# mourisl/centrifuger

Hardware: AMD Instinct MI355X
Metric: classified reads/sec (150 bp) (higher is better)
Workload: dtype u64; 1 GPU; 1.00 Gbp synthetic index (50x5x4 Mbp), 10000000 x 150 bp SE reads per step per GPU, -k 1, inputs resident in HBM; index_bp=1000000000, read_len=150, parallelism=reads sharded over 1 GPU(s), index replicated, no collective

## Files before the change

centrifuger_amd/csrc/cfr_device.hip:

```cpp
#include "cfr_device.hpp"

#include <hipcub/hipcub.hpp>
#include <chrono>

#include <algorithm>
#include <atomic>
#include <functional>
#include <cstdlib>
#include <cstring>
#include <thread>
#include <type_traits>

#include "cfr_hip_util.hpp"
#include "cfr_tail.hpp"
#include "cfr_kernels.hip.inc"

namespace cfr {

namespace {

inline const char *dbg_env(const char *name) {
  static const bool on = [] { const char *g = ::getenv("CFR_DEBUG_ENV"); return g && atoi(g) != 0; }();
  return on ? ::getenv(name) : nullptr;
}
// ... 551 lines not shown
      }
    } catch (const HipError &) {
      (void)hipGetLastError();
      (void)hipStreamSynchronize(stream_);
      for (void *q : tmp_here) temp_free(q);
      if (d_sa) (void)hipFree(d_sa);
      if (d_text_alloc) (void)hipFree(d_text_alloc);
      view_.sa32 = nullptr; view_.sa36 = nullptr; view_.text2 = nullptr; view_.text8 = nullptr; view_.text_min_l = 0;
      memset(&view_.steps, 0, sizeof(view_.steps));
    }
  }
  view_.loc_memo = nullptr;
  view_.memo_shift = 0;
  {
    const bool have_sa_now = have_sa();
    double budget_gb = opt.loc_memo_gb;
    if (budget_gb < 0) {
      budget_gb = fast_load ? 0.0 : 16.0;
      size_t free_b = 0, total_b = 0;
      if (!fast_load && hipMemGetInfo(&free_b, &total_b) == hipSuccess) budget_gb = std::max(have_sa_now ? 0.0 : budget_gb, ((double)free_b - 16e9) / 1e9);
      if (have_sa_now && (double)h.n * 4.0 > budget_gb * 1e9) budget_gb = 0;
    }
    if (const char *e = dbg_env("CFR_LOC_MEMO_GB")) budget_gb = atof(e);
    uint64_t max_val = h.adjusted_sa0;
    for (uint64_t x : h.selected_vals) max_val = std::max(max_val, x);
    if (protein && h.prot.end_marker_bits > 32) max_val = ~0ull;
    const bool fits32 = h.sampled_bits <= 32 && max_val <= 0xffffffffull;
    uint32_t shift = 0;
    while (shift < 8 && (double)((h.n >> shift) + 1) * 4.0 > budget_gb * 1e9) ++shift;
    if (budget_gb > 0 && fits32 && (1u << shift) < (uint32_t)h.sample_rate) try {
      const uint64_t entries = ((h.n - 1) >> shift) + 1;
      uint32_t *d_memo = dev_alloc<uint32_t>(entries);
      const unsigned gm = (unsigned)std::min<uint64_t>((entries + 255) / 256, 1u << 20);
      if (have_sa_now && view_.steps.pos && !(dbg_env("CFR_MEMO_WALK") && atoi(dbg_env("CFR_MEMO_WALK"))))
        k_memo_fill<<<gm, 256, 0, stream_>>>(view_, shift, entries, d_memo);
      else
        k_build_loc_memo<<<gm, 256, 0, stream_>>>(view_, shift, entries, d_memo);
      HIP_CHECK(hipGetLastError());
      HIP_CHECK(hipStreamSynchronize(stream_));
      view_.loc_memo = d_memo;
      view_.memo_shift = shift;
    } catch (const HipError &) { (void)hipGetLastError(); view_.loc_memo = nullptr; view_.memo_shift = 0; }
  }
  lap("locate memo");
  {
    size_t free_b = 0, total_b = 0;
    if (hipMemGetInfo(&free_b, &total_b) == hipSuccess) {
      const double budget = std::min(32e9, 0.4 * (double)free_b);
      piece_bases_max_ = (uint64_t)std::max(2.5e8, budget / 2.7);
    }
  }
  view_.max_entries = (uint64_t)(int64_t)(h.params.max_result * h.params.max_result_per_hit_factor);
  view_.locate_all = (h.params.max_result_per_hit_factor <= 0 || h.params.max_result <= 0) ? 1 : 0;
  d_view_ = dev_alloc<DevView>(1);
  HIP_CHECK(hipMemcpy(d_view_, &view_, sizeof(DevView), hipMemcpyHostToDevice));
}

DeviceIndex::~DeviceIndex() { release(); }

void DeviceIndex::release() {
  (void)hipSetDevice(device_);
  (void)hipDeviceSynchronize();
  for (void *p : owned_) (void)hipFree(p);
  owned_.clear();
  for (void *p : temps_) (void)hipFree(p);
  temps_.clear();
  for (auto &s : slots_) if (s.p) (void)hipFree(s.p);
  slots_.clear();
  if (pinned_) (void)hipHostFree(pinned_);
  pinned_ = nullptr; pinned_cap_ = 0;
  auto drop_event = [](hipEvent_t &e) { if (e) (void)hipEventDestroy(e); e = nullptr; };
  for (auto &set : evs_) for (auto &e : set) drop_event(e);
  for (auto &e : tail_done_) drop_event(e);
  for (auto &e : copy_done_) drop_event(e);
  for (auto &e : h2d_done_) drop_event(e);
  for (auto &e : copied_) drop_event(e);
  for (auto &e : search_done_) drop_event(e);
  for (auto &e : merge_ev_) drop_event(e);
  auto drop_stream = [](hipStream_t &s) { if (s) (void)hipStreamDestroy(s); s = nullptr; };
  drop_stream(tail_stream_);
  drop_stream(search2_stream_);
  if (prep_done_) { (void)hipEventDestroy(prep_done_); prep_done_ = nullptr; }
  drop_stream(h2d_stream_);
  drop_stream(dust_stream_);
  drop_stream(copy_stream_);
  drop_stream(stream_);
}

void *DeviceIndex::temp_alloc(size_t bytes) {
  void *p = nullptr;
  HIP_CHECK(hipMalloc(&p, std::max<size_t>(bytes, 16)));
  temps_.push_back(p);
  return p;
}
void DeviceIndex::temp_free(void *p) {
  if (!p) return;
  auto it = std::find(temps_.begin(), temps_.end(), p);
  if (it != temps_.end()) temps_.erase(it);
  (void)hipFree(p);
}

void DeviceIndex::rank_batch(const char *chars, const uint64_t *pos, const uint8_t *incl, size_t n, uint64_t *out_rank, char *out_access) {
  HIP_CHECK(hipSetDevice(device_));
  if (n == 0) return;
  char *d_c = (char *)scratch(S_P0, n);
  uint64_t *d_p = (uint64_t *)scratch(S_P1, n * 8);
// ... 763 lines not shown
    HIP_CHECK(hipStreamWaitEvent(copy_stream_, tail_done_[par], 0));
    static const bool no_copy = dbg_env("CFR_NO_COPY_OUT") && atoi(dbg_env("CFR_NO_COPY_OUT"));
    if (!no_copy) {
      HIP_CHECK(hipMemcpyAsync(reinterpret_cast<char *>(results) + lo * res_bytes, d_res, cnt * res_bytes, hipMemcpyDeviceToHost, copy_stream_));
      if (extent) HIP_CHECK(hipMemcpyAsync(reinterpret_cast<char *>(matches) + stride * lo * match_bytes, d_match, extent * match_bytes, hipMemcpyDeviceToHost, copy_stream_));
    }
    if (d_flag) HIP_CHECK(hipMemcpyAsync(h_flag, d_flag, kCtlWords * 8, hipMemcpyDeviceToHost, copy_stream_));
    HIP_CHECK(hipEventRecord(copy_done_[par], copy_stream_));
  };
  auto out_buffers = [&](size_t k, uint64_t extent, cfr_result *&d_res, cfr_match *&d_match, hipStream_t st) {
    const int par = (int)(k & 1);
    d_res = (cfr_result *)scratch(par ? S_RESULTS1 : S_RESULTS, std::max(pieces[k].second, sb) * sizeof(cfr_result));
    d_match = (cfr_match *)scratch(par ? S_MATCHES1 : S_MATCHES, (std::max<uint64_t>(extent, stride * sb) + 1) * sizeof(cfr_match));
    if (k >= 2) HIP_CHECK(hipStreamWaitEvent(st, copy_done_[par], 0));
  };

  std::vector<size_t> todo;
  for (size_t k = 0; k < nsub; ++k) todo.push_back(k);
  if (one_launch) {
    unsigned long long *pin = (unsigned long long *)pinned((2 + kCtlWords * kMaxSub + 3 * (kMaxSub + 1)) * 8);
    unsigned long long *pctl = pin + 2;
    for (size_t k = 0; k < kCtlWords * kMaxSub; ++k) pctl[k] = 0;
    if (!pool_cap_) pool_cap_ = std::max<uint64_t>(8ull * sb, 1ull << 20);
    const uint64_t pool_limit = std::max<uint64_t>(256ull * sb, 1ull << 26);
    for (int attempt = 0; attempt < 4 && !todo.empty(); ++attempt) {
      TailEntry *pool_e = (TailEntry *)scratch(S_POOL_E, pool_cap_ * sizeof(TailEntry));
      uint64_t *pool_v = (uint64_t *)scratch(S_POOL_V, pool_cap_ * 8);
      for (size_t k : todo) {
        const size_t lo = pieces[k].first, cnt = pieces[k].second;
        pctl[kCtlWords * k] = 0;
        ev_ = evs_[k];
        if (attempt == 0) { bring_piece(k); pack_piece(k); }
        const int par = tail_overlap ? (int)(k & 1) : 0;
        hipStream_t ts = tail_overlap ? tail_stream_ : stream_;
        hipStream_t ss = two_search && par ? search2_stream_ : stream_;
        search_stream_ = ss;
        if (two_search && par && !prep_waited) { HIP_CHECK(hipEventRecord(prep_done_, stream_)); HIP_CHECK(hipStreamWaitEvent(search2_stream_, prep_done_, 0)); prep_waited = true; }
        if (tail_overlap) HIP_CHECK(hipStreamWaitEvent(ss, tail_done_[par], 0));
        if (pack_rest_pending && k >= 1) { HIP_CHECK(hipStreamWaitEvent(stream_, copied_[0], 0)); pack_rest_pending = false; }
        pre_hit_off_ = hit_all ? hit_all + lo : nullptr;
        pre_hit_base_ = hit_all ? hbase[k] : 0;
        const SearchBuf sbuf = launch_search(d_b1, d_o1 + lo, d_b2, paired ? d_o2 + lo : nullptr, cnt, pt1[k], pt2[k], par);
        pre_hit_off_ = nullptr;
        search_stream_ = nullptr;
        for (int e : {8, 3, 4, 5, 6}) HIP_CHECK(hipEventRecord(ev_[e], ss));
        if (tail_overlap) {
          HIP_CHECK(hipEventRecord(search_done_[par], ss));
          HIP_CHECK(hipStreamWaitEvent(ts, search_done_[par], 0));
        }
        unsigned long long *ctl = (unsigned long long *)scratch((k & 1) ? S_POOLCTL1 : S_POOLCTL, 64);
        cfr_result *d_res;
        cfr_match *d_match;
        out_buffers(k, stride * cnt, d_res, d_match, ts);
        HIP_CHECK(hipMemsetAsync(ctl, 0, 64, ts));
        uint64_t *heavy = team_tail_ ? (uint64_t *)scratch(par ? S_HEAVY1 : S_HEAVY, std::max(sb, cnt) * 32) : nullptr;
        static const uint32_t direct_rows = dbg_env("CFR_HEAVY_DIRECT_ROWS") ? (uint32_t)atoi(dbg_env("CFR_HEAVY_DIRECT_ROWS")) : 64u;
        uint64_t *heavy2 = team_tail_ ? (uint64_t *)scratch(par ? S_HEAVYB1 : S_HEAVYB, std::max(sb, cnt) * 32) : nullptr;
        const unsigned tail_grid = tail_overlap && tail_blocks_per_cu_ ? std::min<unsigned>(grid_for(cnt), (unsigned)(num_cus_ * tail_blocks_per_cu_)) : grid_for(cnt);
        static const bool view_ptr = !(dbg_env("CFR_TAIL_VIEW_PTR") && atoi(dbg_env("CFR_TAIL_VIEW_PTR")) == 0);
        static const bool post_fast = dbg_env("CFR_POST_FAST") && atoi(dbg_env("CFR_POST_FAST")) != 0;
        uint32_t *slow = nullptr;
        unsigned long long *slow_cnt = nullptr;
        unsigned fat_grid = tail_grid;
        static const bool skip_post = dbg_env("CFR_SKIP_POST") && atoi(dbg_env("CFR_SKIP_POST")) != 0;
        if (skip_post) { copy_out(k, d_res, d_match, stride * cnt, ctl + 1, &pctl[kCtlWords * k], ts); if (attempt == 0 && k + 1 < nsub) bring_piece(k + 1); continue; }
        static const int post_fast_last = dbg_env("CFR_POST_FAST_LAST") ? atoi(dbg_env("CFR_POST_FAST_LAST")) : 0;
        if (post_fast && (k + 1 < nsub || post_fast_last || !tail_overlap)) {
          slow = (uint32_t *)scratch(par ? S_SLOW1 : S_SLOW, std::max(sb, cnt) * 4);
          slow_cnt = ctl + 4;
          if (paired) k_post_fast<4><<<tail_grid, kBlock, 0, ts>>>(view_, d_o1 + lo, d_o2 + lo, cnt, sbuf.hit_off, sbuf.raw, sbuf.chain_cnt, d_res, d_match, stride, stride * lo,
                                                               heavy, ctl + 2, heavy2, ctl + 3, direct_rows, slow, slow_cnt);
          else k_post_fast<2><<<tail_grid, kBlock, 0, ts>>>(view_, d_o1 + lo, nullptr, cnt, sbuf.hit_off, sbuf.raw, sbuf.chain_cnt, d_res, d_match, stride, stride * lo,
                                                          heavy, ctl + 2, heavy2, ctl + 3, direct_rows, slow, slow_cnt);
          fat_grid = std::min<unsigned>(grid_for(cnt), (unsigned)(num_cus_ * 2));
        }
        if (paired && view_ptr && d_view_) k_adjust_tail_p<4><<<fat_grid, kBlock, 0, ts>>>(d_view_, d_b1, d_o1 + lo, d_b2, d_o2 + lo, cnt, sbuf.hit_off, sbuf.raw, sbuf.chain_cnt,
                                                                      pool_e, pool_v, ctl, pool_cap_, (uint32_t *)(ctl + 1), d_res, d_match, stride, stride * lo, heavy, ctl + 2, heavy2, ctl + 3, direct_rows, slow, slow_cnt);
        else if (paired) k_adjust_tail<4><<<fat_grid, kBlock, 0, ts>>>(view_, d_b1, d_o1 + lo, d_b2, d_o2 + lo, cnt, sbuf.hit_off, sbuf.raw, sbuf.chain_cnt,
                                                                      pool_e, pool_v, ctl, pool_cap_, (uint32_t *)(ctl + 1), d_res, d_match, stride, stride * lo, heavy, ctl + 2, heavy2, ctl + 3, direct_rows, slow, slow_cnt);
        else k_adjust_tail<2><<<fat_grid, kBlock, 0, ts>>>(view_, d_b1, d_o1 + lo, nullptr, nullptr, cnt, sbuf.hit_off, sbuf.raw, sbuf.chain_cnt,
                                                               pool_e, pool_v, ctl, pool_cap_, (uint32_t *)(ctl + 1), d_res, d_match, stride, stride * lo, heavy, ctl + 2, heavy2, ctl + 3, direct_rows, slow, slow_cnt);
        if (heavy) {
          const unsigned per_cu = (unsigned)(tail_overlap && tail_blocks_per_cu_ ? std::min(5, 2 * tail_blocks_per_cu_) : 5);
          const unsigned hb = std::min<unsigned>((unsigned)((cnt + kTeamsPerBlock - 1) / kTeamsPerBlock), (unsigned)num_cus_ * per_cu);
          const unsigned hb2 = std::min<unsigned>((unsigned)((cnt + kTeams2PerBlock - 1) / kTeams2PerBlock), (unsigned)num_cus_ * std::min(per_cu, 4u));
          if (paired) {
            k_tail_heavy<4, kTeam, kTeamSlots, kTeamsPerBlock, kTeamMaxEntries><<<hb, kTeam * kTeamsPerBlock, 0, ts>>>(
                view_, d_o1 + lo, d_o2 + lo, sbuf.hit_off, sbuf.raw, heavy, ctl + 2, pool_e, pool_v, ctl, pool_cap_, (uint32_t *)(ctl + 1), d_res, d_match, stride, stride * lo, heavy2, ctl + 3);
            k_tail_heavy<4, kTeam2, kTeam2Slots, kTeams2PerBlock, kTeam2MaxEntries><<<hb2, kTeam2 * kTeams2PerBlock, 0, ts>>>(
                view_, d_o1 + lo, d_o2 + lo, sbuf.hit_off, sbuf.raw, heavy2, ctl + 3, pool_e, pool_v, ctl, pool_cap_, (uint32_t *)(ctl + 1), d_res, d_match, stride, stride * lo, nullptr, nullptr);
          } else {
            k_tail_heavy<2, kTeam, kTeamSlots, kTeamsPerBlock, kTeamMaxEntries><<<hb, kTeam * kTeamsPerBlock, 0, ts>>>(
                view_, d_o1 + lo, nullptr, sbuf.hit_off, sbuf.raw, heavy, ctl + 2, pool_e, pool_v, ctl, pool_cap_, (uint32_t *)(ctl + 1), d_res, d_match, stride, stride * lo, heavy2, ctl + 3);
            k_tail_heavy<2, kTeam2, kTeam2Slots, kTeams2PerBlock, kTeam2MaxEntries><<<hb2, kTeam2 * kTeams2PerBlock, 0, ts>>>(
                view_, d_o1 + lo, nullptr, sbuf.hit_off, sbuf.raw, heavy2, ctl + 3, pool_e, pool_v, ctl, pool_cap_, (uint32_t *)(ctl + 1), d_res, d_match, stride, stride * lo, nullptr, nullptr);
          }
        }
        HIP_CHECK(hipGetLastError());
        copy_out(k, d_res, d_match, stride * cnt, ctl + 1, &pctl[kCtlWords * k], ts);
        if (attempt == 0) last_stats.n_chains += cnt * (size_t)(paired ? 4 : 2);
        if (attempt == 0 && k + 1 < nsub) bring_piece(k + 1);
      }
      HIP_CHECK(hipStreamSynchronize(stream_));
      if (two_search) HIP_CHECK(hipStreamSynchronize(search2_stream_));
      HIP_CHECK(hipStreamSynchronize(tail_stream_));
      HIP_CHECK(hipStreamSynchronize(copy_stream_));
      if (attempt == 0) for (size_t k = 0; k < nsub; ++k) { ev_ = evs_[k]; finish_stats(true); }
      if (attempt == 0) {
        unsigned long long hv = 0, slow_reads = 0;
        for (size_t k = 0; k < nsub; ++k) { hv += pctl[kCtlWords * k + 1] + pctl[kCtlWords * k + 2]; slow_reads += pctl[kCtlWords * k + 3]; }
        heavy_frac_ = (double)hv / (double)n;
        last_slow_reads_ = slow_reads; last_team_reads_ = hv;
        if (dbg_env("CFR_POST_STATS")) {
          unsigned long long t1 = 0, t2 = 0;
          for (size_t k = 0; k < nsub; ++k) { t1 += pctl[kCtlWords * k + 1]; t2 += pctl[kCtlWords * k + 2]; }
          fprintf(stderr, "[cfr] post stage of %zu reads: %llu left to k_adjust_tail, %llu folded by small teams, %llu by large teams\n", n, slow_reads, t1, t2);
        }
      }
      std::vector<size_t> again;
      for (size_t k : todo) if (pctl[kCtlWords * k]) again.push_back(k);
      todo.swap(again);
      if (todo.empty() || pool_cap_ >= pool_limit || dbg_env("CFR_POOL_CAP")) break;
      pool_cap_ = std::min(pool_cap_ * 4, pool_limit);
    }
  }
  const bool repeated = one_launch && !todo.empty();

  if (pack_rest_pending) { HIP_CHECK(hipStreamWaitEvent(stream_, copied_[0], 0)); pack_rest_pending = false; }
  for (size_t k : todo) {
    const size_t lo = pieces[k].first, cnt = pieces[k].second;
    ev_ = evs_[k];
    Pipe p;
    run_device_stages(d_b1, d_o1 + lo, d_b2, paired ? d_o2 + lo : nullptr, cnt, pt1[k], pt2[k], true, p, nullptr, fused);
    const uint64_t extent = stride ? stride * cnt : p.nrows;
    if (!stride) {
      if (match_extent) *match_extent = extent;
      if (extent > match_cap) { HIP_CHECK(hipStreamSynchronize(stream_)); throw CapacityError{"match buffer too small"}; }
    }
    TailEntry *entries = (TailEntry *)scratch(S_ENTRIES, (p.nrows + 1) * sizeof(TailEntry));
    cfr_result *d_res;
    cfr_match *d_match;
    out_buffers(k, extent, d_res, d_match, stream_);
    if (fused) k_tail<true><<<grid_for(cnt), kBlock, 0, stream_>>>(view_, cnt, d_o1 + lo, paired ? d_o2 + lo : nullptr, p.hit_off, p.fin_off, p.hits,
                                                                  p.row_off, p.vals, entries, d_res, d_match, stride, stride * lo);
    else k_tail<false><<<grid_for(cnt), kBlock, 0, stream_>>>(view_, cnt, d_o1 + lo, paired ? d_o2 + lo : nullptr, p.fin_off, nullptr, p.hits,
                                                              p.row_off, p.vals, entries, d_res, d_match, stride, stride * lo);
    HIP_CHECK(hipGetLastError());
    copy_out(k, d_res, d_match, extent, nullptr, nullptr, stream_);
  }
  HIP_CHECK(hipStreamSynchronize(stream_));
  HIP_CHECK(hipStreamSynchronize(copy_stream_));
  if (!one_launch) for (size_t k = 0; k < nsub; ++k) { ev_ = evs_[k]; finish_stats(true); }
  if (compact) {
    unsigned long long cntw = 0;
    HIP_CHECK(hipMemcpy(&cntw, wide_side.cnt, 8, hipMemcpyDeviceToHost));
    wide_total_ = cntw;
    const size_t take = (size_t)std::min<unsigned long long>(cntw, kWideSideCap);
    if (take) {
      wide_idx_.resize(take); wide_res_.resize(take); wide_match_.resize(take * stride);
      HIP_CHECK(hipMemcpy(wide_idx_.data(), wide_side.idx, take * 4, hipMemcpyDeviceToHost));
// ... 210 lines not shown
```

centrifuger_amd/csrc/cfr_device.hpp:

```cpp
#pragma once

#include <hip/hip_runtime.h>

#include <cstdint>
#include <string>
#include <utility>
#include <vector>

#include "cfr_index.hpp"

namespace cfr {

struct RankLines { const uint64_t *lines; uint64_t nbits; };
struct RbView {
  RankLines use, plain[3], runs[3];
  uint64_t b;
  uint64_t block_cnt;
  const uint64_t *sel_filter;
  uint32_t filter_rate;
  uint32_t enabled;
};

struct ProtView {
  uint32_t enabled, sigma, bits, endmarker_bits;
  const uint64_t *rec;
  const uint64_t *planes;
  const uint64_t *counts;
  const uint64_t *endmarker;
  uint64_t endmarker_n;
  const uint8_t *code_of;
  uint64_t C[33];
  char list[32];
};

constexpr uint64_t kVirtRow = 1ull << 63;

struct StepView {
  const uint64_t *pos, *val;
  const uint32_t *bucket;
  uint64_t cnt, n;
  uint32_t shift;
};

struct DevView {
  uint64_t n, first_isa, adjusted_sa0;
  uint64_t C[5];
  RbView rb;
  ProtView prot;
  const uint64_t *occ;
  const uint64_t *ftab;
  const uint64_t *ftabx;
  uint32_t ftabx_width;
  uint32_t ftabx_e8;
  const uint64_t *sampled;
  const uint32_t *loc_memo;
  uint32_t memo_shift;
  const uint32_t *sa32;
  const uint32_t *sa36;
  StepView steps;
  const uint64_t *text2;
  const uint8_t *text8;
  uint32_t text_min_l;
  const uint64_t *sel_rows, *sel_vals;
  uint64_t sel_cnt;
  uint32_t last_code, ftab_width, sampled_bits, sample_rate;
  int32_t min_hit_len, score_adjust;
  uint64_t max_entries;
  int32_t locate_all;
  int32_t max_result;
  const uint64_t *tax_parent, *tax_orig, *seq_to_tax;
  const uint8_t *tax_rank;
  const uint32_t *tax_depth;
  uint64_t node_cnt, seq_cnt, tax_root;
  uint64_t secondary_hit_len;
  double secondary_factor;
  uint8_t rank_num[32];
  uint64_t *exp_pool;
  unsigned long long *exp_cursor;
  uint64_t exp_cap;
};

struct TailEntry { uint64_t seq_id, score; int32_t hit_length, k; };

struct HipError { std::string msg; int code; };
struct CapacityError { std::string msg; };
void *host_alloc_pinned(size_t bytes);
void host_free_pinned(void *p);

struct HostSrc { const uint8_t *b1; const uint64_t *o1; const uint8_t *b2; const uint64_t *o2;
                 const uint64_t *p1 = nullptr, *p2 = nullptr; uint64_t *stage1 = nullptr, *stage2 = nullptr; };

class DeviceIndex {
 public:
  DeviceIndex(const HostIndex &h, int device, const cfr_device_options &opt);
  ~DeviceIndex();

  const HostIndex &host() const { return *host_; }
  int device() const { return device_; }
  uint64_t device_bytes() const { return device_bytes_; }
  hipStream_t stream() const { return stream_; }

  void rank_batch(const char *chars, const uint64_t *pos, const uint8_t *incl, size_t n, uint64_t *out_rank, char *out_access);
  void backward_search_batch(const uint8_t *bases, const uint64_t *offsets, const uint32_t *m, size_t n,
                             uint64_t *out_l, uint64_t *out_sp, uint64_t *out_ep);
  void locate_rows(const uint64_t *rows, size_t n, uint64_t *out_val, uint32_t *out_steps);

  void selfcheck(uint64_t out[6]);

  struct BatchOut {
    std::vector<uint64_t> hit_begin;
    std::vector<cfr_hit> hits;
    std::vector<uint64_t> row_begin;
    std::vector<uint64_t> row_vals;
    std::vector<int32_t> read_len;
  };
  void run_batch(const uint8_t *d_bases1, const uint64_t *d_offs1, const uint8_t *d_bases2, const uint64_t *d_offs2,
                 size_t n, uint64_t total1, uint64_t total2, bool want_rows, BatchOut &out);

  void classify_device(const uint8_t *d_bases1, const uint64_t *d_offs1, const uint8_t *d_bases2, const uint64_t *d_offs2,
                       size_t n, uint64_t total1, uint64_t total2, cfr_result *results, cfr_match *matches, size_t match_cap,
                       size_t *match_extent, const struct HostSrc *src = nullptr, bool compact = false);
// ... 34 lines not shown
                  const int8_t *q1, *q2; const int32_t *dec; };
  Merged merge_on_device(const uint8_t *d_b1, const uint64_t *d_o1, const int8_t *d_q1, const uint8_t *d_b2, const uint64_t *d_o2,
                         const int8_t *d_q2, size_t n, uint64_t total1, uint64_t total2, bool want_qual);
  bool merge_ = false, merge_ready_ = false;
  hipEvent_t merge_ev_[2] = {};
  void init(const HostIndex &h, const cfr_device_options &opt);
  void release();
  void *temp_alloc(size_t bytes);
  void temp_free(void *p);
  template <class T> T *dev_alloc(size_t count);
  template <class T> T *upload(const std::vector<T> &v);
  struct Staged { const uint8_t *b1; const uint64_t *o1; const uint8_t *b2; const uint64_t *o2; uint64_t t1, t2; };
  Staged stage_inputs(const uint8_t *b1, const uint64_t *o1, const uint8_t *b2, const uint64_t *o2, size_t n);
  struct Pipe { uint64_t *hit_off, *fin_off, *row_off, *rows, *vals; cfr_hit *hits; uint64_t nhits, nrows; };
  void run_device_stages(const uint8_t *d_b1, const uint64_t *d_o1, const uint8_t *d_b2, const uint64_t *d_o2, size_t n,
                         uint64_t total1, uint64_t total2, bool want_rows, Pipe &p, std::vector<uint64_t> *hit_begin_host,
                         bool fused = false, bool row_space_only = false);
  struct SearchBuf { uint64_t *hit_off; cfr_hit *raw; uint32_t *chain_cnt; uint64_t cap_total; };
  SearchBuf launch_search(const uint8_t *d_b1, const uint64_t *d_o1, const uint8_t *d_b2, const uint64_t *d_o2, size_t n,
                          uint64_t total1, uint64_t total2, int par = 0, bool row_space_only = false);
  bool have_sa() const { return view_.sa32 != nullptr || view_.sa36 != nullptr; }
  bool locate_direct() const { return (view_.loc_memo && view_.memo_shift == 0) || (have_sa() && view_.steps.pos); }
  SearchBuf launch_search_protein(const uint8_t *d_b1, const uint64_t *d_o1, const uint8_t *d_b2, const uint64_t *d_o2, size_t n,
                                  uint64_t total1, uint64_t total2, bool row_space_only = false);
  void launch_post(const SearchBuf &sb, const uint8_t *d_b1, const uint64_t *d_o1, const uint8_t *d_b2, const uint64_t *d_o2, size_t n,
                   bool want_rows, Pipe &p, std::vector<uint64_t> *hit_begin_host, bool fused, hipStream_t st);
  std::vector<std::pair<size_t, size_t>> cut_pieces(size_t n, bool per_read_slots, size_t &sb, uint64_t total_bases = 0) const;
  void dust_on_device(uint8_t *d_bases, const uint64_t *d_offs, size_t n, hipStream_t st);
  void *scratch(size_t slot, size_t bytes);
  void *pinned(size_t bytes);
  void finish_stats(bool want_rows);
  void pack_inputs(const uint8_t *d_b1, uint64_t total1, const uint8_t *d_b2, uint64_t total2, bool pack_now = true);
  void expand_begin();
  bool expand_end();
  uint64_t exp_cap_ = 0;
  int exp_attempt_ = 0;
  uint64_t last_stats_exp_retries_ = 0;
 public:
  uint64_t last_slow_reads_ = 0, last_team_reads_ = 0;
 private:
  int prot_occ_[2] = {0, 0};
  bool one_launch_ready() const { return fused_tail_ && fused_post_ && locate_direct() && !view_.prot.enabled; }

  const HostIndex *host_;
  int device_;
  hipStream_t stream_ = nullptr;
  DevView view_{};
  DevView *d_view_ = nullptr;
  std::vector<void *> owned_, temps_;
  uint64_t device_bytes_ = 0;
  struct Slot { void *p = nullptr; size_t cap = 0; };
  std::vector<Slot> slots_;
  static constexpr size_t kMaxSub = 16;
  hipEvent_t evs_[kMaxSub][9] = {};
  hipEvent_t *ev_ = nullptr;
  hipStream_t copy_stream_ = nullptr, h2d_stream_ = nullptr, tail_stream_ = nullptr, dust_stream_ = nullptr;
  hipStream_t search2_stream_ = nullptr, search_stream_ = nullptr;
  hipEvent_t prep_done_ = nullptr;
  bool two_search_now_ = false;
  hipEvent_t search_done_[2] = {};
  int tail_overlap_mode_ = -1;
  bool overlap_now_ = false, blocks_forced_ = false;
  double heavy_frac_ = 0.0;
  int tail_blocks_per_cu_ = 0;
  hipEvent_t tail_done_[2] = {}, copy_done_[2] = {}, h2d_done_[kMaxSub] = {}, copied_[kMaxSub] = {};
  size_t sub_batch_ = 1250000, taper_floor_ = 262144;
  const uint64_t *prot_o1_base_ = nullptr;
  uint64_t prot_reads_ = 0;
  uint64_t prot_total1_ = 0, prot_total2_ = 0;
  uint64_t piece_bases_max_ = 12000000000ull;
  int num_cus_ = 256, blocks_per_cu_ = 7;
  uint64_t *packed1_ = nullptr, *packed2_ = nullptr;
  uint64_t nblk1_ = 0, nblk2_ = 0;
  double dust_mean_len_ = 0.0;
  bool search_split_default_ = false;
  bool search_v1_ = false, fused_tail_ = true, fused_post_ = true, dust_ = false, team_tail_ = true;
  bool wide_ = false;
  uint64_t pool_cap_ = 0;
  void *pinned_ = nullptr;
  size_t pinned_cap_ = 0;
  const uint64_t *pre_hit_off_ = nullptr;
  uint64_t pre_hit_base_ = 0;
};

}
```

centrifuger_amd/csrc/cfr_kernels.hip.inc:

```
#pragma once

namespace cfr {

constexpr uint64_t kSelFlag = 1ull << 63;
constexpr uint32_t kVirtDeltaShift = 36;
constexpr uint64_t kVirtRowMask = (1ull << kVirtDeltaShift) - 1ull;
constexpr uint32_t kVirtDeltaMax = (1u << 27) - 1u;

struct __attribute__((packed, aligned(4))) U128a4 { uint64_t x, y; };
__device__ __forceinline__ ulonglong2 ld16(const void *p) {
  const U128a4 t = *reinterpret_cast<const U128a4 *>(p);
  return make_ulonglong2(t.x, t.y);
}

typedef uint32_t cfr_u32x4 __attribute__((ext_vector_type(4)));
typedef cfr_u32x4 cfr_u32x4a4 __attribute__((aligned(4)));
__device__ __forceinline__ ulonglong2 ld16_nt(const void *p) {
  const cfr_u32x4 t = __builtin_nontemporal_load(reinterpret_cast<const cfr_u32x4a4 *>(p));
  return make_ulonglong2((uint64_t)t.x | ((uint64_t)t.y << 32), (uint64_t)t.z | ((uint64_t)t.w << 32));
}
#ifndef CFR_GATHER_NT
#define CFR_GATHER_NT 0
#endif
__device__ __forceinline__ ulonglong2 ld16_gather(const void *p) { return CFR_GATHER_NT == 1 ? ld16_nt(p) : ld16(p); }
// ... 568 lines not shown
}
__device__ __forceinline__ uint64_t sampled_read(const DevView &v, uint64_t idx) {
  const uint64_t bit = idx * v.sampled_bits;
  const uint64_t w0 = v.sampled[bit >> 6], w1 = v.sampled[(bit >> 6) + 1];
  const uint32_t sh = (uint32_t)bit & 63u;
  uint64_t x = w0 >> sh;
  if (sh) x |= w1 << (64 - sh);
  return v.sampled_bits >= 64 ? x : (x & ((1ull << v.sampled_bits) - 1));
}

struct __attribute__((packed, aligned(4))) U64a4 { uint64_t x; };
__device__ __forceinline__ uint64_t ld36(const uint32_t *tab, uint64_t i) {
  const uint64_t bit = 36ull * i;
  const uint64_t x = reinterpret_cast<const U64a4 *>(tab + (bit >> 5))->x;
  return (x >> ((uint32_t)bit & 31u)) & 0xfffffffffull;
}
__device__ __forceinline__ void st36_zeroed(uint32_t *tab, uint64_t i, uint64_t val) {
  const uint64_t bit = 36ull * i;
  const uint32_t b = (uint32_t)bit & 63u;
  unsigned long long *t64 = reinterpret_cast<unsigned long long *>(tab) + (bit >> 6);
  atomicOr(t64, (unsigned long long)(val << b));
  if (b > 28u) atomicOr(t64 + 1, (unsigned long long)(val >> (64u - b)));
}
__device__ __forceinline__ uint64_t sa_entry(const DevView &v, uint64_t row) { return v.sa32 ? (uint64_t)v.sa32[row] : ld36(v.sa36, row); }

__global__ void k_ftabx_textpos(DevView v, uint32_t K, uint64_t *table) {
  const uint64_t entries = 1ull << (2 * K);
  for (uint64_t key = (uint64_t)blockIdx.x * blockDim.x + threadIdx.x; key < entries; key += (uint64_t)gridDim.x * blockDim.x) {
    const uint64_t y = table[2 * key + 1];
    if (y != ((1ull << 8) | (uint64_t)K)) continue;
    const uint64_t sp = table[2 * key];
    if (sp == v.first_isa) continue;
    table[2 * key + 1] = kFtabxTextPos | (sa_entry(v, sp) << 16) | y;
  }
}

__device__ __forceinline__ uint64_t steps_value(const StepView &S, uint64_t p) {
  if (p >= S.n) p = S.n - 1;
  const uint64_t b = p >> S.shift;
  uint64_t lo = S.bucket[b], hi = S.bucket[b + 1];
  while (lo < hi) { const uint64_t mid = (lo + hi + 1) >> 1; if (S.pos[mid] <= p) lo = mid; else hi = mid - 1; }
  return S.val[lo];
}
__device__ __forceinline__ uint64_t virt_text_pos(const DevView &v, const cfr_hit &H, uint64_t row) {
  uint32_t m = (uint32_t)H.pad;
  for (uint32_t q = (uint32_t)(row - H.sp); q; --q) m &= m - 1u;
  const uint32_t k = (uint32_t)__ffs((int)m) - 1u;
  return sa_entry(v, (H.sp & kVirtRowMask) + k) - ((H.sp >> kVirtDeltaShift) & (uint64_t)kVirtDeltaMax);
}
__device__ __forceinline__ uint64_t locate_row(const DevView &v, const cfr_hit &H, uint64_t row) {
  if (H.sp & kVirtRow) return steps_value(v.steps, virt_text_pos(v, H, row));
  if (v.loc_memo && v.memo_shift == 0) return (uint64_t)v.loc_memo[row];
  return steps_value(v.steps, sa_entry(v, row));
}

template <bool USE_MEMO = true>
__device__ __forceinline__ uint64_t fm_locate(const DevView &v, uint64_t i, uint32_t &steps) {
  steps = 0;
  if (i & kVirtRow) return steps_value(v.steps, i & ~kVirtRow);
  if (USE_MEMO && !(v.loc_memo && v.memo_shift == 0) && v.steps.pos && (v.sa32 || v.sa36)) return steps_value(v.steps, sa_entry(v, i));
  for (;;) {
    if (USE_MEMO && v.loc_memo && (i & ((1ull << v.memo_shift) - 1)) == 0) return v.loc_memo[i >> v.memo_shift];
    if (i == v.first_isa) return v.adjusted_sa0;
    if (i % v.sample_rate == 0) return sampled_read(v, i / v.sample_rate);
    if (v.prot.enabled) {
      if (i < v.prot.endmarker_n) {
        const uint64_t bit = i * v.prot.endmarker_bits;
        const uint64_t w0 = v.prot.endmarker[bit >> 6], w1 = v.prot.endmarker[(bit >> 6) + 1];
        const uint32_t sh = (uint32_t)bit & 63u;
        uint64_t x = w0 >> sh;
        if (sh) x |= w1 << (64 - sh);
        return v.prot.endmarker_bits >= 64 ? x : (x & ((1ull << v.prot.endmarker_bits) - 1));
      }
      const uint32_t c = prot_access(v.prot, i);
      i = v.prot.C[c] + fm_rank(v, c, i, 1) - 1;
      ++steps;
      continue;
    }
    if (v.rb.enabled) {
      if (v.rb.sel_filter && ((v.rb.sel_filter[(i / v.rb.filter_rate) >> 6] >> ((i / v.rb.filter_rate) & 63u)) & 1ull)) {
        uint64_t val;
        if (sel_lookup(v, i, val)) return val;
      }
      const uint32_t c = rb_access(v.rb, i);
      i = v.C[c] + fm_rank(v, c, i, 1) - 1;
      ++steps;
      continue;
    }
    const uint64_t *rec = occ_rec(v, i);
    const uint32_t h = ((uint32_t)i >> 6) & 1u, j = (uint32_t)i & 63u;
    const ulonglong2 m01 = ld16(rec);
    const ulonglong2 m23 = ld16(rec + 2);
    const ulonglong2 pl = ld16(rec + 4 + 2 * h);
    if (m01.x & kSelFlag) {
      uint64_t val;
      if (sel_lookup(v, i, val)) return val;
    }
    const uint32_t c = (uint32_t)((pl.x >> j) & 1u) | ((uint32_t)((pl.y >> j) & 1u) << 1);
    const uint64_t mid = c == 0 ? m01.x : c == 1 ? m01.y : c == 2 ? m23.x : m23.y;
    i = v.C[c] + occ_count(mid, pl.x, pl.y, c, i, 1) + fm_fix(v, c, i, 1) - 1;
    ++steps;
  }
}

__device__ __forceinline__ uint64_t hit_score(const DevView &v, int32_t l) {
  if (l < v.min_hit_len) return 0;
// ... 789 lines not shown
__device__ __forceinline__ void exp_append(const DevView &v, uint64_t slot, uint64_t *ids, uint64_t cnt, bool as_is) {
  if (!as_is) { sort_u64(ids, cnt); cnt = unique_u64(ids, cnt); }
  if (cnt == 0) return;
  const uint64_t at = (uint64_t)atomicAdd(v.exp_cursor, (unsigned long long)(cnt + 2));
  if (at + cnt + 2 > v.exp_cap) return;
  v.exp_pool[at] = slot;
  v.exp_pool[at + 1] = cnt;
  for (uint64_t j = 0; j < cnt; ++j) v.exp_pool[at + 2 + j] = d_orig_taxid(v, ids[j]);
}

__device__ __forceinline__ void d_tax_expand(const DevView &v, uint64_t *ids, uint64_t cnt, int32_t k, const uint64_t *promoted, uint32_t nm,
                                             uint32_t level, uint64_t *tmp, uint64_t slot0) {
  for (uint64_t i = 0; i < cnt; ++i) if (ids[i] >= v.node_cnt) { exp_append(v, slot0, ids, cnt, true); return; }
  if (k == 1) {
    const uint64_t lca = promoted[0];
    uint64_t m = 0;
    for (uint64_t i = 0; i < cnt; ++i) {
      uint64_t x = ids[i];
      if (x == v.tax_parent[x] || x == lca) continue;
      for (;;) {
        const uint64_t p = v.tax_parent[x];
        if (p == lca || p == v.tax_parent[p]) break;
        x = p;
      }
      tmp[m++] = x;
    }
    exp_append(v, slot0, tmp, m, false);
    return;
  }
  if (level == 0) return;
  for (uint32_t q = 0; q < nm; ++q) {
    uint64_t m = 0;
    for (uint64_t i = 0; i < cnt; ++i) {
      const uint64_t t = d_node_at_level(v, ids[i], level - 1);
      if (t == ~0ull) continue;
      uint64_t x = t, owner = ~0ull;
      while (x != v.tax_parent[x]) {
        x = v.tax_parent[x];
        const uint32_t rn = v.rank_num[v.tax_rank[x]];
        if (rn > level) break;
        if (rn == level) { owner = x; break; }
      }
      if (owner == promoted[q]) tmp[m++] = t;
    }
    exp_append(v, slot0 + q, tmp, m, false);
  }
}

#define CFR_NET8(CE) CE(0,1) CE(2,3) CE(4,5) CE(6,7) CE(0,2) CE(1,3) CE(4,6) CE(5,7) CE(1,2) CE(5,6) CE(0,4) CE(3,7) \
                     CE(1,5) CE(2,6) CE(1,4) CE(3,6) CE(2,4) CE(3,5) CE(3,4)

struct TailFold { uint64_t best, second, best_len, second_len; };

template <class HitAt>
__device__ __forceinline__ bool tail_fold_small(const DevView &v, const HitAt &hit_at, uint64_t nh, bool mix,
                                                TailFold &F, uint64_t (&skey)[8], uint64_t (&ssc)[8], uint32_t &ne_out) {
  uint64_t key[8], sc[8];
  int32_t ln[8];
#pragma unroll
  for (int e = 0; e < 8; ++e) { key[e] = ~0ull; sc[e] = 0; ln[e] = 0; }
  uint32_t ne = 0;
  uint64_t prev_id = 0, prev_score = 0;
  int32_t prev_len = 0;
  cfr_hit P;
  P.sp = 0; P.ep = 1; P.l = 0; P.strand = 0; P.offset = 0; P.pad = 0;
  for (uint64_t h = 0; h < nh; ++h) {
    const cfr_hit H = hit_at(h);
    if (H.l < v.min_hit_len) { P = H; continue; }
    const uint64_t range = H.ep - H.sp + 1;
    if (range > 8 || !(range <= v.max_entries || v.locate_all)) return false;
    uint64_t x[8];
#pragma unroll
    for (int q = 0; q < 8; ++q) x[q] = (uint64_t)q < range ? locate_row(v, H, H.sp + q) : ~0ull;
#define CFR_CE(i, j) { const uint64_t lo_ = x[i] < x[j] ? x[i] : x[j], hi_ = x[i] < x[j] ? x[j] : x[i]; x[i] = lo_; x[j] = hi_; }
    CFR_NET8(CFR_CE)
#undef CFR_CE
    const uint64_t score = hit_score(v, H.l);
    const uint64_t kk = (uint64_t)((H.strand + 1) / 2);
    bool adjacent = false;
    if (!mix && h > 0 && H.ep == H.sp) adjacent = P.ep == P.sp && P.strand == H.strand && P.offset + P.l + 1 == H.offset;
    bool overflow = false;
#pragma unroll
    for (int q = 0; q < 8; ++q) {
      const uint64_t id = x[q];
      const bool live = id != ~0ull && (q == 0 || id != x[q > 0 ? q - 1 : 0]);
      if (live) {
        const uint64_t want = (kk << 32) | id;
        uint32_t idx = ne;
#pragma unroll
        for (int e = 0; e < 8; ++e) if (key[e] == want) idx = (uint32_t)e;
        const bool created = idx == ne;
        if (created && ne == 8) overflow = true;
        else {
          uint64_t s_old = 0;
          int32_t l_old = 0;
#pragma unroll
          for (int e = 0; e < 8; ++e) if ((uint32_t)e == idx) { s_old = sc[e]; l_old = ln[e]; }
          uint64_t s_new;
          int32_t l_new;
          if (adjacent && id == prev_id) {
            prev_len += H.l;
            const uint64_t merged = hit_score(v, prev_len);
            s_new = s_old - prev_score + merged;
            prev_score = merged;
            l_new = l_old + H.l;
          } else {
            s_new = created ? score : s_old + score;
            l_new = created ? H.l : l_old + H.l;
            if (H.ep == H.sp) { prev_id = id; prev_score = score; prev_len = H.l; }
          }
#pragma unroll
          for (int e = 0; e < 8; ++e) if ((uint32_t)e == idx) { key[e] = want; sc[e] = s_new; ln[e] = l_new; }
          if (created) ++ne;
        }
      }
    }
    if (overflow) return false;
    P = H;
  }
#define CFR_CE(i, j) { const bool sw_ = key[i] > key[j]; \
    const uint64_t k_ = key[i], s_ = sc[i]; const int32_t l_ = ln[i]; \
    key[i] = sw_ ? key[j] : k_; sc[i] = sw_ ? sc[j] : s_; ln[i] = sw_ ? ln[j] : l_; \
    key[j] = sw_ ? k_ : key[j]; sc[j] = sw_ ? s_ : sc[j]; ln[j] = sw_ ? l_ : ln[j]; }
  CFR_NET8(CFR_CE)
#undef CFR_CE
  uint64_t best = 0, second = 0, best_len = 0, second_len = 0;
#pragma unroll
  for (int e = 0; e < 8; ++e) if ((uint32_t)e < ne) {
    if (sc[e] > best) { second = best; second_len = best_len; best = sc[e]; best_len = (uint64_t)(int64_t)ln[e]; }
    else if (sc[e] > second) { second = sc[e]; second_len = (uint64_t)(int64_t)ln[e]; }
  }
  F.best = best; F.second = second; F.best_len = best_len; F.second_len = second_len;
#pragma unroll
  for (int e = 0; e < 8; ++e) { skey[e] = key[e]; ssc[e] = sc[e]; }
  ne_out = ne;
  return true;
}

__device__ __forceinline__ uint64_t tail_small_ids(const DevView &v, const TailFold &F, const uint64_t (&skey)[8], const uint64_t (&ssc)[8],
                                                   uint32_t sne, uint64_t (&bid)[8], uint32_t &nb_out) {
  const bool take_second = F.second_len >= v.secondary_hit_len && F.second < F.best && F.second >= (uint64_t)(v.secondary_factor * (double)F.best);
  uint32_t nbr = 0, nb_best = 0;
#pragma unroll
  for (int pass = 0; pass < 2; ++pass) {
    const uint64_t target = pass == 0 ? F.best : F.second;
    if (pass == 0 || take_second) {
#pragma unroll
      for (int e = 0; e < 8; ++e) if ((uint32_t)e < sne && ssc[e] == target) {
        const uint64_t id = skey[e] & 0xffffffffull;
        bool seen = false;
#pragma unroll
        for (int q = 0; q < 8; ++q) if ((uint32_t)q < nbr && bid[q] == id) seen = true;
        if (!seen) {
#pragma unroll
          for (int q = 0; q < 8; ++q) if ((uint32_t)q == nbr) bid[q] = id;
          ++nbr;
        }
      }
    }
    if (pass == 0) nb_best = nbr;
  }
  nb_out = nbr;
  return take_second ? F.second : (nb_best > 1 ? F.best : F.second);
}

template <bool MEMO, class HitAt>
__device__ __forceinline__ void tail_fold_general(const DevView &v, const HitAt &hit_at, uint64_t nh, bool mix, uint64_t *vals_base,
                                                  uint64_t *row_vals, const uint64_t *row_off_h, TailEntry *E, uint64_t *best_ids,
                                                  TailFold &F, uint64_t &nb, uint64_t &sec_out) {
  uint64_t fused_off = 0;
  uint64_t ne = 0;
// ... 2661 lines not shown
```

Measured before the change: 873.2 million reads/s.

## Batch locate lookups for the first post-stage hits in lockstep through shared memory

```diff
diff --git a/centrifuger_amd/csrc/cfr_device.hip b/centrifuger_amd/csrc/cfr_device.hip
--- a/centrifuger_amd/csrc/cfr_device.hip
+++ b/centrifuger_amd/csrc/cfr_device.hip
@@ -627,6 +627,7 @@
   }
   view_.max_entries = (uint64_t)(int64_t)(h.params.max_result * h.params.max_result_per_hit_factor);
   view_.locate_all = (h.params.max_result_per_hit_factor <= 0 || h.params.max_result <= 0) ? 1 : 0;
+  view_.post_lockstep = !(dbg_env("CFR_POST_LOCKSTEP") && atoi(dbg_env("CFR_POST_LOCKSTEP")) == 0) ? 1u : 0u;
   d_view_ = dev_alloc<DevView>(1);
   HIP_CHECK(hipMemcpy(d_view_, &view_, sizeof(DevView), hipMemcpyHostToDevice));
 }
@@ -1496,6 +1497,8 @@
         cfr_result *d_res;
         cfr_match *d_match;
         out_buffers(k, stride * cnt, d_res, d_match, ts);
+        static const bool timeline = dbg_env("CFR_STEP_TIMELINE") && atoi(dbg_env("CFR_STEP_TIMELINE")) != 0;
+        if (timeline && attempt == 0) HIP_CHECK(hipEventRecord(ev_[9], ts));
         HIP_CHECK(hipMemsetAsync(ctl, 0, 64, ts));
         uint64_t *heavy = team_tail_ ? (uint64_t *)scratch(par ? S_HEAVY1 : S_HEAVY, std::max(sb, cnt) * 32) : nullptr;
         static const uint32_t direct_rows = dbg_env("CFR_HEAVY_DIRECT_ROWS") ? (uint32_t)atoi(dbg_env("CFR_HEAVY_DIRECT_ROWS")) : 64u;
@@ -1550,6 +1553,11 @@
       HIP_CHECK(hipStreamSynchronize(tail_stream_));
       HIP_CHECK(hipStreamSynchronize(copy_stream_));
       if (attempt == 0) for (size_t k = 0; k < nsub; ++k) { ev_ = evs_[k]; finish_stats(true); }
+      if (attempt == 0 && dbg_env("CFR_STEP_TIMELINE") && atoi(dbg_env("CFR_STEP_TIMELINE")) != 0 && !dbg_env("CFR_SKIP_POST")) {
+        auto at = [&](size_t k, int e) { float t = 0; (void)hipEventElapsedTime(&t, evs_[0][1], evs_[k][e]); return t; };
+        for (size_t k = 0; k < nsub; ++k)
+          fprintf(stderr, "[cfr] timeline sub-batch %zu: search %.3f .. %.3f  post %.3f .. %.3f ms\n", k, at(k, 1), at(k, 2), at(k, 9), at(k, 7));
+      }
       if (attempt == 0) {
         unsigned long long hv = 0, slow_reads = 0;
         for (size_t k = 0; k < nsub; ++k) { hv += pctl[kCtlWords * k + 1] + pctl[kCtlWords * k + 2]; slow_reads += pctl[kCtlWords * k + 3]; }
diff --git a/centrifuger_amd/csrc/cfr_device.hpp b/centrifuger_amd/csrc/cfr_device.hpp
--- a/centrifuger_amd/csrc/cfr_device.hpp
+++ b/centrifuger_amd/csrc/cfr_device.hpp
@@ -67,6 +67,7 @@
   int32_t min_hit_len, score_adjust;
   uint64_t max_entries;
   int32_t locate_all;
+  uint32_t post_lockstep;
   int32_t max_result;
   const uint64_t *tax_parent, *tax_orig, *seq_to_tax;
   const uint8_t *tax_rank;
@@ -207,7 +208,7 @@
   struct Slot { void *p = nullptr; size_t cap = 0; };
   std::vector<Slot> slots_;
   static constexpr size_t kMaxSub = 16;
-  hipEvent_t evs_[kMaxSub][9] = {};
+  hipEvent_t evs_[kMaxSub][10] = {};
   hipEvent_t *ev_ = nullptr;
   hipStream_t copy_stream_ = nullptr, h2d_stream_ = nullptr, tail_stream_ = nullptr, dust_stream_ = nullptr;
   hipStream_t search2_stream_ = nullptr, search_stream_ = nullptr;
diff --git a/centrifuger_amd/csrc/cfr_kernels.hip.inc b/centrifuger_amd/csrc/cfr_kernels.hip.inc
--- a/centrifuger_amd/csrc/cfr_kernels.hip.inc
+++ b/centrifuger_amd/csrc/cfr_kernels.hip.inc
@@ -644,6 +644,73 @@
   if (H.sp & kVirtRow) return steps_value(v.steps, virt_text_pos(v, H, row));
   if (v.loc_memo && v.memo_shift == 0) return (uint64_t)v.loc_memo[row];
   return steps_value(v.steps, sa_entry(v, row));
+}
+
+template <int N>
+__device__ __forceinline__ void locate_rows_lockstep(const DevView &v, const uint64_t (&row)[N], const uint32_t (&delta)[N], uint32_t virt,
+                                                     uint32_t (&id)[N], bool &wide) {
+  const bool memo_all = v.loc_memo && v.memo_shift == 0;
+  wide = false;
+  if (!((v.sa32 || v.sa36) && v.steps.pos)) {
+#pragma unroll
+    for (int q = 0; q < N; ++q) id[q] = v.loc_memo[row[q]];
+    return;
+  }
+  const StepView &S = v.steps;
+  const uint32_t by_memo = memo_all ? ~virt : 0u;
+  uint64_t p[N];
+  if (v.sa32) {
+#pragma unroll
+    for (int q = 0; q < N; ++q) p[q] = (uint64_t)(((by_memo >> q) & 1u) ? v.loc_memo : v.sa32)[row[q]];
+  } else {
+#pragma unroll
+    for (int q = 0; q < N; ++q) p[q] = ld36(v.sa36, ((by_memo >> q) & 1u) ? 0ull : row[q]);
+    if (memo_all) {
+      uint32_t w[N];
+#pragma unroll
+      for (int q = 0; q < N; ++q) w[q] = v.loc_memo[((by_memo >> q) & 1u) ? row[q] : 0ull];
+#pragma unroll
+      for (int q = 0; q < N; ++q) if ((by_memo >> q) & 1u) p[q] = (uint64_t)w[q];
+    }
+  }
+  uint32_t lo[N], hi[N];
+#pragma unroll
+  for (int q = 0; q < N; ++q) {
+    if (!((by_memo >> q) & 1u)) {
+      p[q] -= (uint64_t)delta[q];
+      if (p[q] >= S.n) p[q] = S.n - 1;
+    }
+  }
+#pragma unroll
+  for (int q = 0; q < N; ++q) {
+    const uint64_t b = ((by_memo >> q) & 1u) ? 0ull : p[q] >> S.shift;
+    lo[q] = S.bucket[b]; hi[q] = S.bucket[b + 1];
+  }
+#pragma unroll
+  for (int q = 0; q < N; ++q) if ((by_memo >> q) & 1u) hi[q] = lo[q];
+  for (;;) {
+    bool any = false;
+#pragma unroll
+    for (int q = 0; q < N; ++q) any |= lo[q] < hi[q];
+    if (!any) break;
+    uint64_t pm[N];
+#pragma unroll
+    for (int q = 0; q < N; ++q) pm[q] = S.pos[(uint32_t)(((uint64_t)lo[q] + hi[q] + 1) >> 1)];
+#pragma unroll
+    for (int q = 0; q < N; ++q) {
+      const uint32_t mid = (uint32_t)(((uint64_t)lo[q] + hi[q] + 1) >> 1);
+      if (lo[q] < hi[q]) { if (pm[q] <= p[q]) lo[q] = mid; else hi[q] = mid - 1; }
+    }
+  }
+  uint64_t val[N];
+#pragma unroll
+  for (int q = 0; q < N; ++q) val[q] = S.val[lo[q]];
+#pragma unroll
+  for (int q = 0; q < N; ++q) {
+    const bool m = (by_memo >> q) & 1u;
+    wide |= !m && (val[q] >> 32) != 0;
+    id[q] = m ? (uint32_t)p[q] : (uint32_t)val[q];
+  }
 }
 
 template <bool USE_MEMO = true>
@@ -1539,9 +1606,68 @@
 
 struct TailFold { uint64_t best, second, best_len, second_len; };
 
+constexpr int kPostBatchRows = 8, kPostBatchHits = 4, kPostBatchLanes = 256;
+__device__ __forceinline__ uint32_t sel4(uint32_t j, uint32_t a, uint32_t b, uint32_t c, uint32_t d) { return j == 0 ? a : j == 1 ? b : j == 2 ? c : d; }
+__device__ __forceinline__ uint64_t sel4(uint32_t j, uint64_t a, uint64_t b, uint64_t c, uint64_t d) { return j == 0 ? a : j == 1 ? b : j == 2 ? c : d; }
+
+template <class HitAt>
+__device__ __forceinline__ uint32_t tail_gather_rows(const DevView &v, const HitAt &hit_at, uint64_t nh, uint32_t *s_ids) {
+  if (!v.post_lockstep || nh == 0) return 0;
+  uint64_t sp[kPostBatchHits];
+  uint32_t pad[kPostBatchHits], cnt[kPostBatchHits];
+  bool leaves = false;
+#pragma unroll
+  for (int j = 0; j < kPostBatchHits; ++j) {
+    const cfr_hit H = hit_at((uint64_t)j < nh ? (uint64_t)j : nh - 1);
+    const uint64_t range = H.ep - H.sp + 1;
+    const bool counts = (uint64_t)j < nh && H.l >= v.min_hit_len;
+    leaves |= counts && (range > 8 || !(range <= v.max_entries || v.locate_all));
+    sp[j] = H.sp; pad[j] = (uint32_t)H.pad;
+    cnt[j] = counts ? (uint32_t)(range < 9 ? range : 9) : 0u;
+  }
+  if (leaves) return 0;
+  uint32_t nbh = 0, total = 0;
+  bool open = true;
+#pragma unroll
+  for (int j = 0; j < kPostBatchHits; ++j) {
+    open = open && (uint64_t)j < nh && total + cnt[j] <= (uint32_t)kPostBatchRows;
+    if (open) { total += cnt[j]; nbh = (uint32_t)j + 1u; } else cnt[j] = 0;
+  }
+  if (total == 0) return 0;
+  uint64_t row[kPostBatchRows];
+  uint32_t delta[kPostBatchRows], virt = 0;
+  uint32_t hc = 0, left = 0, r = 0, m = 0, d_last = 0;
+  uint64_t cur = 0, row_last = 0;
+  bool v_last = false;
+#pragma unroll
+  for (int q = 0; q < kPostBatchRows; ++q) {
+    while (left == 0 && hc < nbh) {
+      left = sel4(hc, cnt[0], cnt[1], cnt[2], cnt[3]); cur = sel4(hc, sp[0], sp[1], sp[2], sp[3]); m = sel4(hc, pad[0], pad[1], pad[2], pad[3]);
+      r = 0; ++hc;
+    }
+    if (left) {
+      v_last = (cur & kVirtRow) != 0;
+      const uint32_t k = v_last ? (uint32_t)__ffs((int)m) - 1u : r;
+      row_last = (v_last ? (cur & kVirtRowMask) : cur) + k;
+      d_last = v_last ? (uint32_t)((cur >> kVirtDeltaShift) & (uint64_t)kVirtDeltaMax) : 0u;
+      m &= m - 1u; ++r; --left;
+    }
+    row[q] = row_last; delta[q] = d_last; virt |= (v_last ? 1u : 0u) << q;
+  }
+  uint32_t g[kPostBatchRows];
+  bool wide;
+  locate_rows_lockstep<kPostBatchRows>(v, row, delta, virt, g, wide);
+#pragma unroll
+  for (int q = 0; q < kPostBatchRows; ++q) s_ids[q * kPostBatchLanes + threadIdx.x] = g[q];
+  return wide ? 0u : nbh;
+}
+
 template <class HitAt>
 __device__ __forceinline__ bool tail_fold_small(const DevView &v, const HitAt &hit_at, uint64_t nh, bool mix,
                                                 TailFold &F, uint64_t (&skey)[8], uint64_t (&ssc)[8], uint32_t &ne_out) {
+  __shared__ uint32_t s_ids[kPostBatchRows * kPostBatchLanes];
+  const uint32_t nbh = tail_gather_rows(v, hit_at, nh, s_ids);
+  uint32_t gpos = 0;
   uint64_t key[8], sc[8];
   int32_t ln[8];
 #pragma unroll
@@ -1549,23 +1675,32 @@
   uint32_t ne = 0;
   uint64_t prev_id = 0, prev_score = 0;
   int32_t prev_len = 0;
-  cfr_hit P;
-  P.sp = 0; P.ep = 1; P.l = 0; P.strand = 0; P.offset = 0; P.pad = 0;
+  bool p_unique = false;
+  int32_t p_strand = 0, p_next = 1;
   for (uint64_t h = 0; h < nh; ++h) {
     const cfr_hit H = hit_at(h);
-    if (H.l < v.min_hit_len) { P = H; continue; }
+    if (H.l < v.min_hit_len) { p_unique = H.ep == H.sp; p_strand = H.strand; p_next = H.offset + H.l + 1; continue; }
     const uint64_t range = H.ep - H.sp + 1;
     if (range > 8 || !(range <= v.max_entries || v.locate_all)) return false;
     uint64_t x[8];
-#pragma unroll
-    for (int q = 0; q < 8; ++q) x[q] = (uint64_t)q < range ? locate_row(v, H, H.sp + q) : ~0ull;
+    if (h < nbh) {
+#pragma unroll
+      for (int q = 0; q < 8; ++q) {
+        const uint32_t got = s_ids[((gpos + (uint32_t)q) & (uint32_t)(kPostBatchRows - 1)) * kPostBatchLanes + threadIdx.x];
+        x[q] = (uint64_t)q < range ? (uint64_t)got : ~0ull;
+      }
+      gpos += (uint32_t)range;
+    } else {
+#pragma unroll
+      for (int q = 0; q < 8; ++q) x[q] = (uint64_t)q < range ? locate_row(v, H, H.sp + q) : ~0ull;
+    }
 #define CFR_CE(i, j) { const uint64_t lo_ = x[i] < x[j] ? x[i] : x[j], hi_ = x[i] < x[j] ? x[j] : x[i]; x[i] = lo_; x[j] = hi_; }
     CFR_NET8(CFR_CE)
 #undef CFR_CE
     const uint64_t score = hit_score(v, H.l);
     const uint64_t kk = (uint64_t)((H.strand + 1) / 2);
     bool adjacent = false;
-    if (!mix && h > 0 && H.ep == H.sp) adjacent = P.ep == P.sp && P.strand == H.strand && P.offset + P.l + 1 == H.offset;
+    if (!mix && h > 0 && H.ep == H.sp) adjacent = p_unique && p_strand == H.strand && p_next == H.offset;
     bool overflow = false;
 #pragma unroll
     for (int q = 0; q < 8; ++q) {
@@ -1603,7 +1738,7 @@
       }
     }
     if (overflow) return false;
-    P = H;
+    p_unique = H.ep == H.sp; p_strand = H.strand; p_next = H.offset + H.l + 1;
   }
 #define CFR_CE(i, j) { const bool sw_ = key[i] > key[j]; \
     const uint64_t k_ = key[i], s_ = sc[i]; const int32_t l_ = ln[i]; \
```

Measured after the change: 863.2 million reads/s. -1.1%, worse.
